# JuliaLinearAlgebra/ArnoldiMethod.jl

Measured on AMD Instinct MI355X. Metric: arnoldi_iters_per_sec, higher is better.
Workload: dtype f64

## Files before the change

arnoldimethod.jl_amd/csrc/ks_csr_layout.hpp:

```cpp
#pragma once

#include <algorithm>
#include <climits>
#include <cmath>
#include <cstring>
#include <unordered_map>
#include <vector>

#include "ks_host_defs.hpp"

namespace {

enum class CbMode {
  None,
  Allowed,
  IsColumnBlock,
  DistributedRowBlock
};

struct FormatRequest {
  bool format_set = false;
  std::string format;
  bool ptr64 = false;
  int sell_sigma = 1;
// ... 35 lines not shown
  bool sell_keeps_dict() const { return format != "sell"; }
};

template <class D> struct CsrHost {
  int64_t nrows, nnz;
  const std::vector<int64_t>& rp;
  const std::vector<int32_t>& ci;
  const std::vector<D>& vv;
};

template <class D> struct CsrPlan {
  int layout = -1;
  bool ptr64 = false;
  double bytes_per_nnz = 0.0, aux_bytes = 0.0;
  int nstencil = 0, nstencil_local = 0, stencil_mask_bytes = 1;
  std::vector<int32_t> sdelta;
  std::vector<D> sval;
  std::vector<uint8_t> mask8;
  std::vector<uint32_t> mask32;
  int ndvi = 0, dvi_unroll = 8, dvi_rpt = 1;
  std::vector<uint8_t> codes;
  std::vector<int32_t> ddelta;
  std::vector<D> dval;
  int ndict = 0;
  std::vector<D> dict;
  std::vector<int32_t> packed;
  int nslices = 0, sell_un = 8;
  int64_t sell_entries = 0;
  std::vector<int64_t> sliceptr;
  std::vector<int32_t> sell_col, sell_perm;
  std::vector<D> sell_val;
  std::vector<CsrPlan<D>> cblocks;
  std::vector<char> cb_from_ghost;
  std::vector<int64_t> cb_bounds;
  int cb_rpt = 0, cb_ni = 0;
  std::vector<int64_t> sub_rp;
  std::vector<int32_t> sub_ci;
  std::vector<D> sub_vv;
  int ni = 7, nblk = 0, nlong = 0;
  bool row_gather = false;
  std::vector<int64_t> blkptr;
  std::vector<int32_t> blkrow, blkpart, lrow, lfirst;
};

template <class D> struct DviDict {
  bool ok = true;
  std::vector<uint8_t> codes;
  std::vector<int32_t> delta;
  std::vector<D> val;
  int64_t max_row = 0;
  std::vector<uint8_t> local_used = std::vector<uint8_t>(256, 0);
};

template <class D> DviDict<D> build_dvi_dict(const CsrHost<D>& A) {
  struct Key {
    uint64_t a, b;
    int64_t d;
    bool operator==(const Key& o) const { return a == o.a && b == o.b && d == o.d; }
  };
  struct KeyHash {
    size_t operator()(const Key& k) const {
      return std::hash<uint64_t>()((k.a * 0x9E3779B97F4A7C15ull ^ k.b) + (uint64_t)k.d * 0xC2B2AE3D27D4EB4Full);
    }
  };
  DviDict<D> t;
  std::unordered_map<Key, int, KeyHash> index;
  t.codes.resize((size_t)A.nnz);
  Key ckey[8];
  int cid[8], ncache = 0, cnext = 0;
  for (int64_t r = 0; r < A.nrows && t.ok; ++r) {
    t.max_row = std::max(t.max_row, A.rp[r + 1] - A.rp[r]);
    for (int64_t p = A.rp[r]; p < A.rp[r + 1]; ++p) {
      Key k{0, 0, (int64_t)A.ci[p] - r};
      std::memcpy(&k, &A.vv[p], sizeof(D));
      bool hit = false;
      for (int q = 0; q < ncache; ++q)
        if (ckey[q] == k) { t.codes[p] = (uint8_t)cid[q]; hit = true; break; }
      if (hit) { if (A.ci[p] < A.nrows) t.local_used[t.codes[p]] = 1; continue; }
      auto it = index.find(k);
      int id;
      if (it == index.end()) {
        if (t.delta.size() == 256) { t.ok = false; break; }
        id = (int)t.delta.size();
        index.emplace(k, id);
        t.delta.push_back((int32_t)k.d);
        t.val.push_back(A.vv[p]);
      } else {
        id = it->second;
      }
      t.codes[p] = (uint8_t)id;
      if (A.ci[p] < A.nrows) t.local_used[id] = 1;
      ckey[cnext] = k;
      cid[cnext] = id;
      cnext = (cnext + 1) & 7;
      if (ncache < 8) ++ncache;
    }
  }
  return t;
}

template <class D> bool plan_stencil(const CsrHost<D>& A, const DviDict<D>& t, CsrPlan<D>& P) {
  const int ns = (int)t.delta.size();
  std::vector<uint32_t> succ((size_t)ns, 0u);
  for (int64_t r = 0; r < A.nrows; ++r)
    for (int64_t p = A.rp[r] + 1; p < A.rp[r + 1]; ++p) succ[t.codes[p - 1]] |= 1u << t.codes[p];
  std::vector<int> indeg((size_t)ns, 0), order;
  for (int a = 0; a < ns; ++a)
    for (int b = 0; b < ns; ++b)
      if (succ[a] >> b & 1u) indeg[b]++;
  std::vector<char> done((size_t)ns, 0);
  for (int it = 0; it < ns; ++it) {
    int pick = -1;
    for (int a = 0; a < ns; ++a)
      if (!done[a] && indeg[a] == 0) { pick = a; break; }
    if (pick < 0) return false;
    done[pick] = 1;
    order.push_back(pick);
    for (int b = 0; b < ns; ++b)
      if (succ[pick] >> b & 1u) indeg[b]--;
  }
  std::vector<int> slot((size_t)ns, 0);
  for (int k = 0; k < ns; ++k) slot[order[k]] = k;
  const int mbytes = ns <= 8 ? 1 : 4;
  std::vector<uint8_t> m8;
  std::vector<uint32_t> m32;
  if (mbytes == 1) m8.assign((size_t)A.nrows, 0); else m32.assign((size_t)A.nrows, 0u);
  for (int64_t r = 0; r < A.nrows; ++r) {
    uint32_t m = 0;
    int last = -1;
    for (int64_t p = A.rp[r]; p < A.rp[r + 1]; ++p) {
      const int k = slot[t.codes[p]];
      if (k <= last) return false;
      last = k;
      m |= 1u << k;
    }
    if (mbytes == 1) m8[r] = (uint8_t)m; else m32[r] = m;
  }
  P.nstencil = ns;
  P.nstencil_local = ns;
  for (int k = ns - 1; k >= 0 && !t.local_used[order[k]]; --k) P.nstencil_local = k;
  P.stencil_mask_bytes = mbytes;
  for (int k = 0; k < ns; ++k) {
    P.sdelta.push_back(t.delta[order[k]]);
    P.sval.push_back(t.val[order[k]]);
  }
  P.mask8 = std::move(m8);
  P.mask32 = std::move(m32);
  P.layout = KS_LAYOUT_STENCIL;
  P.bytes_per_nnz = (double)mbytes * (double)A.nrows / (double)A.nnz;
  P.aux_bytes = 0.0;
  return true;
}

template <class D> void plan_dvi(const CsrHost<D>& A, DviDict<D>&& t, const FormatRequest& req, CsrPlan<D>& P) {
  P.ndvi = (int)t.delta.size();
  P.dvi_unroll = t.max_row <= 4 ? 4 : 8;
  P.dvi_rpt = req.dvi_rpt;
  P.codes = std::move(t.codes);
  P.ddelta = std::move(t.delta);
  P.dval = std::move(t.val);
  P.layout = KS_LAYOUT_DVI;
  P.bytes_per_nnz = 1.0;
  P.aux_bytes = (P.ptr64 ? 8.0 : 4.0) * (double)(A.nrows + 1);
}

template <class D> void build_vi_dict(const CsrHost<D>& A, CsrPlan<D>& P) {
  struct Key {
    uint64_t a, b;
    bool operator==(const Key& o) const { return a == o.a && b == o.b; }
  };
  struct KeyHash {
    size_t operator()(const Key& k) const { return std::hash<uint64_t>()(k.a * 0x9E3779B97F4A7C15ull ^ k.b); }
  };
  std::unordered_map<Key, int, KeyHash> index;
  Key last_key{0, 0};
  int last_id = 0;
  bool ok = true;
  std::vector<D> dict;
  std::vector<int32_t> packed((size_t)A.nnz);
  for (int64_t p = 0; p < A.nnz && ok; ++p) {
    Key k{0, 0};
    std::memcpy(&k, &A.vv[p], sizeof(D));
    int id;
    if (p > 0 && k == last_key) {
      id = last_id;
    } else {
      auto it = index.find(k);
      if (it == index.end()) {
        if (dict.size() == 256) { ok = false; break; }
        id = (int)dict.size();
        index.emplace(k, id);
        dict.push_back(A.vv[p]);
      } else {
        id = it->second;
      }
      last_key = k;
      last_id = id;
    }
    if (A.ci[p] >= (1 << 24)) { ok = false; break; }
    packed[p] = (int32_t)(((uint32_t)id << 24) | (uint32_t)A.ci[p]);
  }
  if (!ok) return;
  P.dict = std::move(dict);
  P.packed = std::move(packed);
  P.ndict = (int)P.dict.size();
}

template <class D> bool plan_sell(const CsrHost<D>& A, const FormatRequest& req, CsrPlan<D>& P) {
  const std::vector<int64_t>& rp = A.rp;
  const int64_t nrows = A.nrows;
  const int sigma = req.sell_sigma;
  std::vector<int32_t> perm;
  if (sigma > 1) {
    perm.resize((size_t)nrows);
    for (int64_t i = 0; i < nrows; ++i) perm[i] = (int32_t)i;
    for (int64_t w0 = 0; w0 < nrows; w0 += sigma) {
      const int64_t w1 = std::min<int64_t>(nrows, w0 + sigma);
      std::stable_sort(perm.begin() + w0, perm.begin() + w1,
                       [&](int32_t x_, int32_t y_) { return rp[x_ + 1] - rp[x_] > rp[y_ + 1] - rp[y_]; });
    }
  }
  auto row_at = [&](int64_t pos) { return sigma > 1 ? (int64_t)perm[pos] : pos; };
  const int64_t nsl = (nrows + 63) / 64;
  std::vector<int64_t> sp((size_t)nsl + 1, 0);
  int64_t wmax = 0;
  for (int64_t sl = 0; sl < nsl; ++sl) {
    int64_t w = 0;
    for (int64_t pos = sl * 64; pos < std::min<int64_t>(nrows, sl * 64 + 64); ++pos) {
      const int64_t r = row_at(pos);
      w = std::max(w, rp[r + 1] - rp[r]);
    }
    wmax = std::max(wmax, w);
    sp[sl + 1] = sp[sl] + 64 * w;
  }
  const int64_t padded = sp[nsl];
  if (!(req.force_sell() || (double)padded <= 1.15 * (double)A.nnz + 64.0)) return false;
  KS_REQUIRE(padded < ((int64_t)1 << 40), KS_ERR_ARGUMENT, "sliced-ELLPACK padding explodes: use KS_SPMV_FORMAT=csr");
  if (padded >= (int64_t)2147483647) P.ptr64 = true;
  const bool vi = P.ndict > 0;
  P.sell_col.assign((size_t)padded, -1);
  P.sell_val.resize(vi ? 0 : (size_t)padded);
  for (int64_t sl = 0; sl < nsl; ++sl)
    for (int64_t pos = sl * 64; pos < std::min<int64_t>(nrows, sl * 64 + 64); ++pos) {
      const int64_t r = row_at(pos);
      const int64_t lane = pos - sl * 64;
      for (int64_t p = rp[r], k = 0; p < rp[r + 1]; ++p, ++k) {
        const int64_t q = sp[sl] + k * 64 + lane;
        P.sell_col[q] = vi ? P.packed[p] : A.ci[p];
        if (!vi) P.sell_val[q] = A.vv[p];
      }
    }
  P.nslices = (int)nsl;
  P.sell_un = wmax <= 4 ? 4 : 8;
  P.sell_entries = padded;
  P.sliceptr = std::move(sp);
  P.sell_perm = std::move(perm);
  P.layout = vi ? KS_LAYOUT_SELL_VI : KS_LAYOUT_SELL;
  P.bytes_per_nnz = (vi ? 4.0 : 4.0 + sizeof(D)) * (double)padded / (double)A.nnz;
  P.aux_bytes = (P.ptr64 ? 8.0 : 4.0) * (double)(nsl + 1) + (sigma > 1 ? 4.0 * (double)nrows : 0.0);
  return true;
}

template <class D> void plan_row_blocks(const CsrHost<D>& A, const FormatRequest& req, CsrPlan<D>& P) {
  const std::vector<int64_t>& rp = A.rp;
  const int64_t nrows = A.nrows;
  constexpr int kBlock = ksd::kBlock;
  const int nimax = (int)(ksd::kSpmvCapBytes / (kBlock * sizeof(D)));
  std::vector<int64_t> tile_nnz;
  for (int64_t r0 = 0; r0 < nrows; r0 += ksd::kSpmvRows) tile_nnz.push_back(rp[std::min<int64_t>(nrows, r0 + ksd::kSpmvRows)] - rp[r0]);
  int64_t t90 = 0;
  if (!tile_nnz.empty()) {
    const size_t k = (tile_nnz.size() - 1) * 9 / 10;
    std::nth_element(tile_nnz.begin(), tile_nnz.begin() + k, tile_nnz.end());
    t90 = tile_nnz[k];
  }
  const int need = (int)((t90 + kBlock - 1) / kBlock);
  int ni = need <= 4 ? 4 : need <= 7 ? 7 : need <= 8 ? 8 : need <= 12 ? 12 : 16;
  if (req.ni != INT_MIN) ni = req.ni;
  if (ni != 4 && ni != 7 && ni != 8 && ni != 12 && ni != 16) ni = 16;
  ni = std::min(ni, nimax);
  P.ni = ni;
  {
    int64_t pairs = 0, close = 0;
    const int64_t stride = std::max<int64_t>(1, nrows / 65536);
    for (int64_t r = 0; r + 1 < nrows; r += stride) {
      if (rp[r + 1] == rp[r] || rp[r + 2] == rp[r + 1]) continue;
      ++pairs;
      const int64_t d = (int64_t)A.ci[rp[r + 1]] - (int64_t)A.ci[rp[r]];
      if (d >= -16 && d <= 16) ++close;
    }
    P.row_gather = req.row_gather >= 0 ? req.row_gather != 0 : (pairs > 0 && 2 * close >= pairs);
  }
  const int64_t cap = (int64_t)ni * kBlock;
  std::vector<int64_t>& bp = P.blkptr;
  std::vector<int32_t>&br = P.blkrow, &part = P.blkpart, &lrow = P.lrow, &lfirst = P.lfirst;
  bp = {0};
  br = {0};
  lfirst = {0};
  int64_t r = 0;
  while (r < nrows) {
    const int64_t first = rp[r + 1] - rp[r];
    if (first > cap) {
      for (int64_t q = rp[r]; q < rp[r + 1]; q += cap) {
        part.push_back((int32_t)lfirst.back() + (int32_t)((q - rp[r]) / cap));
        br.push_back((int32_t)(r + 1));
        bp.push_back(std::min(q + cap, rp[r + 1]));
// ... 172 lines not shown
```

arnoldimethod.jl_amd/csrc/ks_operators.hpp:

```cpp
#pragma once
struct ks_operator {
  ks_ctx* ctx = nullptr;
  int64_t n_local = 0, nnz = 0;
  int dtype = KS_F64;
  bool async_capable = true;
  double bytes_per_nnz = 0.0;
  double aux_bytes = 0.0;
  int layout = -1;
  double in_scale = 1.0;
  bool shift_store_cacheable = false;
  virtual ~ks_operator() = default;
  virtual void apply(const void* x, void* y, const DevState* st) = 0;
  virtual void apply_shifted(const void* x, void* y, double theta_re, double theta_im, double sigma, int64_t ld, const DevState* st);
};

namespace {

template <class D> struct CsrOp : ks_operator {
  void* rowptr = nullptr;
  bool ptr64 = false;
  int32_t* colidx = nullptr;
  D* val = nullptr;
  void* blkptr = nullptr;
  int32_t* blkrow = nullptr;
  int nblk = 0;
  std::vector<std::unique_ptr<CsrOp<D>>> cblocks;
  std::vector<char> cb_from_ghost;
  int cb_rpt = 0, cb_ni = 0;
  int ni = 7;
  bool row_gather = false;
  int nlong = 0;
  int32_t* blkpart = nullptr;
  D* lpart = nullptr;
  int32_t* lrow = nullptr;
  int32_t* lfirst = nullptr;
  int nstencil = 0;
  int stencil_mask_bytes = 1;
  void* smask = nullptr;
  void* smask2 = nullptr;
  ksd::StencilDict<D> sdict{};
  int nstencil_local = 0;
  mutable bool split_said = false;
  void* sliceptr = nullptr;
  int32_t* sperm = nullptr;
  int nslices = 0;
  int sell_un = 8;
  int64_t sell_entries = 0;
  int ndict = 0;
  int ndvi = 0;
  uint8_t* codes = nullptr;
  int32_t* ddelta = nullptr;
  int dvi_unroll = 8;
  int dvi_rpt = 1;
  Halo<D> halo;

  ~CsrOp() override {
    (void)hipFree(rowptr); (void)hipFree(colidx); (void)hipFree(val); (void)hipFree(blkptr); (void)hipFree(blkrow); (void)hipFree(smask); (void)hipFree(sliceptr); (void)hipFree(sperm); (void)hipFree(blkpart); (void)hipFree(lpart); (void)hipFree(lrow); (void)hipFree(lfirst);
    (void)hipFree(codes); (void)hipFree(ddelta);
  }
  void launch_csr_blocks(const D* x, D* y, const DevState* st, const D* yacc, int plain_store, ksd::ShiftArg<D> shift = ksd::ShiftArg<D>{}) {
    hipStream_t s = ctx->stream;
    auto go = [&](auto ip_tag) {
      using IP = decltype(ip_tag);
      auto launch = [&](auto ni_tag) {
        constexpr int NI = decltype(ni_tag)::value;
        if constexpr ((size_t)NI * kBlock * sizeof(D) <= (size_t)ksd::kSpmvCapBytes)
          ksd::k_spmv_csr<D, IP, false, NI><<<nblk, kBlock, 0, s>>>(static_cast<const IP*>(blkptr), blkrow, static_cast<const IP*>(rowptr), colidx, val, x,
                                                                    nullptr, y, n_local, nblk, st, nullptr, 0, 0, nullptr, nullptr, yacc, plain_store,
                                                                    ksd::HaloFused{}, ksd::HaloArgs{}, ksd::P2pDev{}, env_int("KS_SPMV_CSR_NT", 1) != 0, row_gather,
                                                                    plain_store ? ksd::ShiftArg<D>{} : shift);
        else
          throw KsError{KS_ERR_INTERNAL, "CSR row blocks of " + std::to_string(NI) + " x 256 entries exceed the LDS budget of this element type"};
      };
      switch (ni) {
        case 4: launch(std::integral_constant<int, 4>{}); break;
        case 7: launch(std::integral_constant<int, 7>{}); break;
        case 8: launch(std::integral_constant<int, 8>{}); break;
        case 12: launch(std::integral_constant<int, 12>{}); break;
        default: launch(std::integral_constant<int, 16>{}); break;
      }
    };
    if (ptr64) go(int64_t{});
    else go(int32_t{});
  }
  bool shift_on = false;
  D shift_theta{};
  double shift_sigma = 1.0;
  bool shift_plain() const {
    static const int env = env_int("KS_SHIFT_PLAIN", -1);
    return env >= 0 ? env != 0 : shift_store_cacheable;
  }
  static bool march_on() {
    return env_int("KS_STENCIL_MARCH", 1) != 0;
  }
  int march_slots(int ntiles) const {
    const int env = env_int("KS_MARCH_S", 0);
    int S = 192;
    if (env > 0) S = env;
    else {
      int64_t P = 0;
      for (int k = 0; k < nstencil; ++k) P = std::max<int64_t>(P, std::llabs((long long)sdict.delta[k]));
      const int64_t per = P / 512 + 1;
      if (per >= 16 && per <= 224) S = (int)(per * ((160 + per - 1) / per)) <= 224 ? (int)(per * ((160 + per - 1) / per)) : (int)per;
    }
    S = std::min(S, std::max(1, (ntiles + 7) / 8));
    return S;
  }
  void launch_march(const D* x, D* y, int nt, const DevState* st, hipStream_t s) const {
    if constexpr (std::is_same<D, double>::value) {
      const int sh = shift_on ? (1 | (shift_plain() ? 2 : 0)) : 0;
      const uint16_t* m2 = static_cast<const uint16_t*>(smask2);
      const int G = 8 * march_slots(nt);
      int kown = -1;
      for (int k = 0; k < nstencil; ++k)
        if (sdict.delta[k] == 0) kown = k;
      auto go = [&](auto ns_tag, auto ko_tag) {
        ksd::k_spmv_stencil_march<decltype(ns_tag)::value, decltype(ko_tag)::value><<<G, kBlock, 0, s>>>(m2, sdict, x, y, n_local, nt, st, sh, shift_theta, shift_sigma);
      };
      const int window = env_int("KS_MARCH_WINDOW", 1);
      if (window && nstencil == 7 && kown == 3) {
        bool shape = std::llabs((long long)sdict.delta[0]) > 256 && std::llabs((long long)sdict.delta[6]) > 256;
        unsigned odd = 0;
        for (int k = 1; k <= 5; ++k) {
          shape = shape && std::llabs((long long)sdict.delta[k]) <= 256;
          if (sdict.delta[k] & 1) odd |= 1u << k;
        }
        const int zmarch = env_int("KS_MARCH_Z", 1), zr_env = env_int("KS_MARCH_ZR", 0);
        const int64_t Pz = sdict.delta[6];
        if (shape && zmarch && sdict.delta[0] == -Pz && (Pz & 1) == 0 && Pz >= 8 * 8 * 512) {
          const int nzp = (int)((n_local + Pz - 1) / Pz), cmax = (int)(((Pz + 511) / 512 + 7) / 8);
          int nzr = zr_env > 0 ? zr_env : std::max(1, (288 + cmax / 2) / cmax);
          nzr = std::max(1, std::min(nzr, nzp / 4));
          if (nzp >= 8) {
            auto gz = [&](auto odd_tag) {
              ksd::k_spmv_stencil_marchz<7, 0x3eu, decltype(odd_tag)::value, 3, 0, 6><<<8 * cmax * nzr, kBlock, 0, s>>>(m2, sdict, x, y, n_local, nzr, st, sh, shift_theta, shift_sigma);
            };
            if (odd == 0x14u) gz(std::integral_constant<unsigned, 0x14u>{});
            else if (odd == 0x36u) gz(std::integral_constant<unsigned, 0x36u>{});
            else gz(std::integral_constant<unsigned, 0x3eu>{});
            return;
          }
        }
        if (shape) {
          auto gw = [&](auto odd_tag) {
            ksd::k_spmv_stencil_marchw<7, 0x3eu, decltype(odd_tag)::value, 3><<<G, kBlock, 0, s>>>(m2, sdict, x, y, n_local, nt, st, sh, shift_theta, shift_sigma);
          };
          if (odd == 0x14u) gw(std::integral_constant<unsigned, 0x14u>{});
          else if (odd == 0x36u) gw(std::integral_constant<unsigned, 0x36u>{});
          else gw(std::integral_constant<unsigned, 0x3eu>{});
          return;
        }
      }
      using M1 = std::integral_constant<int, -1>;
      if (nstencil == 7 && kown == 3) go(std::integral_constant<int, 7>{}, std::integral_constant<int, 3>{});
      else if (nstencil == 5 && kown == 2) go(std::integral_constant<int, 5>{}, std::integral_constant<int, 2>{});
      else if (nstencil == 3 && kown == 1) go(std::integral_constant<int, 3>{}, std::integral_constant<int, 1>{});
      else switch (nstencil) {
        case 1: go(std::integral_constant<int, 1>{}, M1{}); break;
        case 2: go(std::integral_constant<int, 2>{}, M1{}); break;
        case 3: go(std::integral_constant<int, 3>{}, M1{}); break;
        case 4: go(std::integral_constant<int, 4>{}, M1{}); break;
        case 5: go(std::integral_constant<int, 5>{}, M1{}); break;
        case 6: go(std::integral_constant<int, 6>{}, M1{}); break;
        case 7: go(std::integral_constant<int, 7>{}, M1{}); break;
        default: go(std::integral_constant<int, 8>{}, M1{}); break;
      }
    }
  }
  ksd::ShiftArg<D> shift_arg() const {
    ksd::ShiftArg<D> a;
    a.on = shift_on ? 1 : 0;
    a.theta = shift_theta;
    a.sigma = shift_sigma;
    return a;
  }
  void apply_shifted(const void* xv, void* yv, double tre, double tim, double sigma, int64_t ld, const DevState* st) override {
    const int fuse = env_int("KS_SHIFT_FUSED", 1);
    const bool fused = fuse && n_local > 0 && nlong == 0;
    if (!fused) { ks_operator::apply_shifted(xv, yv, tre, tim, sigma, ld, st); return; }
    shift_on = true;
    if constexpr (sizeof(D) == 8) shift_theta = tre; else shift_theta = D{tre, tim};
    shift_sigma = sigma;
    try { apply(xv, yv, st); } catch (...) { shift_on = false; throw; }
    shift_on = false;
  }
  void apply(const void* xv, void* yv, const DevState* st) override {
    const D* x = static_cast<const D*>(xv);
    D* y = static_cast<D*>(yv);
    hipStream_t s = ctx->stream;
    const typename Halo<D>::Begun begun = halo.begin(x, st, n_local > 0 && cblocks.empty() && ndvi == 0 && nslices == 0);
    const ksd::HaloFused& hf = begun.hf;
    const D* xg = begun.xg;
    if (n_local > 0 && !cblocks.empty()) {
      ProfScope ps(ctx, KSP_SPMV, (double)nnz * bytes_per_nnz + aux_bytes + 2.0 * sizeof(D) * n_local);
      if (cb_rpt) {
        ksd::CbArgs<D> a{};
        a.nb = (int)cblocks.size();
        for (int b = 0; b < a.nb; ++b) {
          a.rowptr[b] = static_cast<const int32_t*>(cblocks[b]->rowptr);
          a.colidx[b] = cblocks[b]->colidx;
          a.val[b] = cblocks[b]->val;
          a.xb[b] = (!cb_from_ghost.empty() && cb_from_ghost[b]) ? xg : nullptr;
        }
        const int nt = (int)((n_local + (int64_t)kBlock * cb_rpt - 1) / ((int64_t)kBlock * cb_rpt));
        auto go = [&](auto ni_tag, auto rpt_tag) {
          constexpr int NI = decltype(ni_tag)::value, RPT = decltype(rpt_tag)::value;
          if constexpr ((size_t)NI * kBlock * sizeof(D) <= (size_t)ksd::kSpmvCapBytes)
            ksd::k_spmv_csr_cb<D, NI, RPT><<<nt, kBlock, 0, s>>>(a, x, y, n_local, nt, st, shift_arg());
          else
            throw KsError{KS_ERR_INTERNAL, "column-blocked CSR: LDS depth exceeds the budget of this element type"};
        };
        auto by_rpt = [&](auto ni_tag) {
          switch (cb_rpt) {
            case 1: go(ni_tag, std::integral_constant<int, 1>{}); break;
            case 2: go(ni_tag, std::integral_constant<int, 2>{}); break;
            case 4: go(ni_tag, std::integral_constant<int, 4>{}); break;
            case 8: go(ni_tag, std::integral_constant<int, 8>{}); break;
            default: go(ni_tag, std::integral_constant<int, 16>{}); break;
          }
        };
        if (cb_ni == 8) by_rpt(std::integral_constant<int, 8>{});
        else by_rpt(std::integral_constant<int, 16>{});
        KS_HIP(hipGetLastError());
        return;
      }
      for (size_t b = 0; b < cblocks.size(); ++b) cblocks[b]->launch_csr_blocks(x, y, st, b > 0 ? y : nullptr, b + 1 < cblocks.size() ? 1 : 0, shift_arg());
      KS_HIP(hipGetLastError());
      return;
    }
    if (n_local > 0) {
      ProfScope ps(ctx, KSP_SPMV, (double)nnz * bytes_per_nnz + aux_bytes + 2.0 * sizeof(D) * n_local);
      const uint32_t* hseq = nullptr;
      auto with_ip = [&](auto f) {
        if (ptr64) f(int64_t{});
        else f(int32_t{});
      };
      if (nstencil > 0 && halo.plan.nghost == 0 && smask2 && n_local >= 2 && env_int("KS_STENCIL_PAIRS", 1)) {
        const int nt = (int)(((n_local + 1) / 2 + kBlock - 1) / kBlock);
        if constexpr (std::is_same<D, double>::value) {
          if (stencil_mask_bytes == 1 && nstencil <= 8 && march_on()) {
            launch_march(x, y, nt, st, s);
            KS_HIP(hipGetLastError());
            return;
          }
        }
        if (stencil_mask_bytes == 1)
          ksd::k_spmv_stencil2<D, uint16_t><<<nt, kBlock, 0, s>>>(static_cast<const uint16_t*>(smask2), sdict, nstencil, x, y, n_local, nt, st, shift_on ? (1 | (shift_plain() ? 2 : 0)) : 0, shift_theta, shift_sigma);
        else
          ksd::k_spmv_stencil2<D, uint64_t><<<nt, kBlock, 0, s>>>(static_cast<const uint64_t*>(smask2), sdict, nstencil, x, y, n_local, nt, st, shift_on ? (1 | (shift_plain() ? 2 : 0)) : 0, shift_theta, shift_sigma);
        KS_HIP(hipGetLastError());
        return;
      }
      if (nstencil > 0 && halo.plan.nghost > 0 && !halo.p2p && smask2 && (stencil_mask_bytes == 1 || stencil_mask_bytes == 4) && n_local >= 2 * kBlock) {
        if constexpr (std::is_same<D, double>::value) {
          static const int split_env = env_int("KS_DIST_SPLIT", 1);
          const int nt1 = (int)((n_local + kBlock - 1) / kBlock);
          const int nlow = (int)((halo.plan.ghost_lo_end + kBlock - 1) / kBlock), first_high = (int)(halo.plan.ghost_hi_begin / kBlock);
          const int nhigh = nt1 - first_high;
          if (split_env && env_int("KS_STENCIL_PAIRS", 1) && nlow <= first_high && 4 * (nlow + nhigh) <= nt1 && nlow + nhigh > 0) {
            const int nt2 = (int)(((n_local + 1) / 2 + kBlock - 1) / kBlock);
            static const int split_dbg = env_int("KS_DIST_SPLIT_DEBUG", 0);
            if (split_dbg && !split_said) {
              split_said = true;
              std::fprintf(stderr, "[split] rows %lld: paired kernel on all of them (%d of %d slots), ghost-aware kernel on %d + %d boundary tiles of %d\n", (long long)n_local, nstencil_local, nstencil, nlow, nhigh, nt1);
            }
            const int shf = shift_on ? (1 | (shift_plain() ? 2 : 0)) : 0;
            ksd::HaloFused h0{};
            const int nsl = nstencil_local >= 1 ? nstencil_local : nstencil;
            if (stencil_mask_bytes == 1) {
              ksd::k_spmv_stencil2<D, uint16_t><<<nt2, kBlock, 0, s>>>(static_cast<const uint16_t*>(smask2), sdict, nsl, x, y, n_local, nt2, st, shf, shift_theta, shift_sigma);
              ksd::k_spmv_stencil<D, uint8_t, 1><<<nlow + nhigh, kBlock, 0, s>>>(static_cast<const uint8_t*>(smask), sdict, nstencil, x, xg, y, n_local,
                                                                                std::max<int64_t>(halo.plan.nghost, 0), nlow + nhigh, st, h0, halo.hargs, ctx->p2p.dev, shift_on ? 1 : 0,
                                                                                shift_theta, shift_sigma, nlow, first_high - nlow);
            } else {
              ksd::k_spmv_stencil2<D, uint64_t><<<nt2, kBlock, 0, s>>>(static_cast<const uint64_t*>(smask2), sdict, nsl, x, y, n_local, nt2, st, shf, shift_theta, shift_sigma);
              ksd::k_spmv_stencil<D, uint32_t, 1><<<nlow + nhigh, kBlock, 0, s>>>(static_cast<const uint32_t*>(smask), sdict, nstencil, x, xg, y, n_local,
                                                                                 std::max<int64_t>(halo.plan.nghost, 0), nlow + nhigh, st, h0, halo.hargs, ctx->p2p.dev, shift_on ? 1 : 0,
                                                                                 shift_theta, shift_sigma, nlow, first_high - nlow);
            }
            KS_HIP(hipGetLastError());
            return;
          }
        }
// ... 117 lines not shown
    KS_HIP(hipGetLastError());
  }
};

struct HostCallbackOp : ks_operator {
  ks_host_apply_fn fn = nullptr;
  void* user = nullptr;
  void* xh = nullptr;
  void* yh = nullptr;
  ~HostCallbackOp() override { (void)hipHostFree(xh); (void)hipHostFree(yh); }
  void apply(const void* x, void* y, const DevState*) override {
    const size_t bytes = (size_t)n_local * (dtype == KS_F64 ? 8 : 16);
    KS_HIP(hipMemcpyAsync(xh, x, bytes, hipMemcpyDeviceToHost, ctx->stream));
    KS_HIP(hipStreamSynchronize(ctx->stream));
    const int64_t nd = n_local * (dtype == KS_F64 ? 1 : 2);
    if (in_scale != 1.0) {
      double* xd = static_cast<double*>(xh);
      for (int64_t i = 0; i < nd; ++i) xd[i] *= in_scale;
    }
    const int rc = fn(user, xh, yh);
    KS_REQUIRE(rc == 0, KS_ERR_OPERATOR, "host operator callback returned " + std::to_string(rc));
    if (in_scale != 1.0) {
      const double back = 1.0 / in_scale;
      double* yd = static_cast<double*>(yh);
      for (int64_t i = 0; i < nd; ++i) yd[i] *= back;
    }
    KS_HIP(hipMemcpyAsync(y, yh, bytes, hipMemcpyHostToDevice, ctx->stream));
  }
};

struct DeviceCallbackOp : ks_operator {
  ks_device_apply_fn fn = nullptr;
  void* user = nullptr;
  void apply(const void* x, void* y, const DevState*) override {
    const int rc = fn(user, x, y, (void*)ctx->stream);
    KS_REQUIRE(rc == 0, KS_ERR_OPERATOR, "device operator callback returned " + std::to_string(rc));
  }
};

template <class I> inline int64_t idx_at(const void* p, int64_t i) { return (int64_t) static_cast<const I*>(p)[i]; }

template <class D>
void build_csr_host(int64_t nrows, int64_t ncols, int64_t nnz, const void* ptr, const void* idx, const void* val,
                    int layout, int base, int itype, std::vector<int64_t>& rp, std::vector<int32_t>& ci,
                    std::vector<D>& vv) {
  auto P = [&](int64_t i) { return (itype == KS_I32 ? idx_at<int32_t>(ptr, i) : idx_at<int64_t>(ptr, i)) - base; };
  auto J = [&](int64_t i) { return (itype == KS_I32 ? idx_at<int32_t>(idx, i) : idx_at<int64_t>(idx, i)) - base; };
  const D* v = static_cast<const D*>(val);
  KS_REQUIRE(nrows < (int64_t)2147483647 && ncols < (int64_t)2147483647, KS_ERR_ARGUMENT, "matrix order must fit int32");
  {
    const int64_t np = (layout == KS_CSR ? nrows : ncols);
    int64_t prev = P(0);
    KS_REQUIRE(prev == 0, KS_ERR_ARGUMENT, layout == KS_CSR ? "row pointer does not match nnz" : "column pointer does not match nnz");
    for (int64_t i = 1; i <= np; ++i) {
      const int64_t cur = P(i);
      KS_REQUIRE(cur >= prev && cur <= nnz, KS_ERR_ARGUMENT, "pointer array is not monotone within [0, nnz]");
      prev = cur;
    }
    KS_REQUIRE(prev == nnz, KS_ERR_ARGUMENT, layout == KS_CSR ? "row pointer does not match nnz" : "column pointer does not match nnz");
  }
  rp.assign(nrows + 1, 0);
  ci.resize(nnz);
  vv.resize(nnz);
  if (layout == KS_CSR) {
    for (int64_t i = 0; i <= nrows; ++i) rp[i] = P(i);
    for (int64_t p = 0; p < nnz; ++p) {
      const int64_t c = J(p);
      KS_REQUIRE(c >= 0 && c < ncols, KS_ERR_ARGUMENT, "column index out of range");
      ci[p] = (int32_t)c;
      vv[p] = v[p];
    }
  } else {
    for (int64_t p = 0; p < nnz; ++p) {
      const int64_t r = J(p);
      KS_REQUIRE(r >= 0 && r < nrows, KS_ERR_ARGUMENT, "row index out of range");
      rp[r + 1]++;
    }
    for (int64_t i = 0; i < nrows; ++i) rp[i + 1] += rp[i];
    std::vector<int64_t> fill(rp.begin(), rp.end() - 1);
    for (int64_t c = 0; c < ncols; ++c)
      for (int64_t p = P(c); p < P(c + 1); ++p) {
        const int64_t r = J(p);
        const int64_t q = fill[r]++;
        ci[q] = (int32_t)c;
        vv[q] = v[p];
      }
  }
}

inline void build_csr_dist_host(int64_t nrows, int64_t nghost, int64_t nnz, const int64_t* rowptr, const int32_t* colidx,
                                std::vector<int64_t>& rp, std::vector<int32_t>& ci) {
  KS_REQUIRE(nrows < (int64_t)2147483647 && nghost < (int64_t)2147483647 - nrows, KS_ERR_ARGUMENT, "local-extended column range must fit int32");
  rp.resize(nrows + 1);
  KS_REQUIRE(rowptr[0] == 0 && rowptr[nrows] == nnz, KS_ERR_ARGUMENT, "row pointer does not match nnz");
  for (int64_t i = 0; i <= nrows; ++i) {
    KS_REQUIRE(i == 0 || (rowptr[i] >= rowptr[i - 1] && rowptr[i] <= nnz), KS_ERR_ARGUMENT, "pointer array is not monotone within [0, nnz]");
    rp[i] = rowptr[i];
  }
  ci.assign(colidx, colidx + nnz);
  for (int64_t p = 0; p < nnz; ++p)
    KS_REQUIRE(ci[p] >= 0 && ci[p] < nrows + nghost, KS_ERR_ARGUMENT, "local-extended column index out of range");
}

inline void* upload_ptr(const std::vector<int64_t>& v, bool ptr64) {
  void* d = nullptr;
  const size_t cnt = v.size();
  if (ptr64) {
    KS_HIP(hipMalloc(&d, std::max<size_t>(cnt * 8, 16)));
    KS_HIP(hipMemcpy(d, v.data(), cnt * 8, hipMemcpyHostToDevice));
  } else {
    std::vector<int32_t> t(v.begin(), v.end());
    KS_HIP(hipMalloc(&d, std::max<size_t>(cnt * 4, 16)));
    KS_HIP(hipMemcpy(d, t.data(), cnt * 4, hipMemcpyHostToDevice));
  }
  return d;
}

template <class T> T* upload_vec(const T* v, size_t cnt, size_t pad, bool zero = false) {
  void* d = nullptr;
  KS_HIP(hipMalloc(&d, (cnt + pad) * sizeof(T)));
  if (zero) KS_HIP(hipMemset(d, 0, (cnt + pad) * sizeof(T)));
  if (cnt) KS_HIP(hipMemcpy(d, v, cnt * sizeof(T), hipMemcpyHostToDevice));
  return static_cast<T*>(d);
}
template <class T> T* upload_vec(const std::vector<T>& v, size_t pad, bool zero = false) { return upload_vec(v.data(), v.size(), pad, zero); }

template <class D>
CsrOp<D>* upload(ks_ctx* ctx, const CsrPlan<D>& P, int64_t nrows, int64_t nnz, const std::vector<int64_t>& rp, const std::vector<int32_t>& ci,
                 const std::vector<D>& vv) {
  auto op = std::make_unique<CsrOp<D>>();
  op->ctx = ctx;
  op->n_local = nrows;
  op->nnz = nnz;
  op->dtype = sizeof(D) == 8 ? KS_F64 : KS_C64;
  op->layout = P.layout;
  op->ptr64 = P.ptr64;
  op->bytes_per_nnz = P.bytes_per_nnz;
  op->aux_bytes = P.aux_bytes;
  op->ndict = P.ndict;
  constexpr size_t kPad16 = 16 / sizeof(D);
  switch (P.layout) {
    case KS_LAYOUT_STENCIL: {
      op->nstencil = P.nstencil;
      op->nstencil_local = P.nstencil_local;
      op->stencil_mask_bytes = P.stencil_mask_bytes;
      for (int k = 0; k < ksd::kStencilSlots; ++k) {
        op->sdict.delta[k] = k < P.nstencil ? P.sdelta[k] : 0;
        op->sdict.val[k] = k < P.nstencil ? P.sval[k] : D{};
      }
      const size_t pad = (size_t)(round_up(nrows + 2, 8) - nrows);
      if (P.stencil_mask_bytes == 1) op->smask = upload_vec(P.mask8, pad, true);
      else op->smask = upload_vec(P.mask32, pad, true);
      op->smask2 = op->smask;
      break;
    }
    case KS_LAYOUT_DVI:
      op->ndvi = P.ndvi;
      op->dvi_unroll = P.dvi_unroll;
      op->dvi_rpt = P.dvi_rpt;
      op->rowptr = upload_ptr(rp, P.ptr64);
      op->codes = upload_vec(P.codes, 64, true);
      op->ddelta = upload_vec(P.ddelta, 256 - P.ddelta.size());
      op->val = upload_vec(P.dval, 256 - P.dval.size());
      break;
    case KS_LAYOUT_SELL:
    case KS_LAYOUT_SELL_VI:
      op->nslices = P.nslices;
      op->sell_un = P.sell_un;
      op->sell_entries = P.sell_entries;
      op->sliceptr = upload_ptr(P.sliceptr, P.ptr64);
      op->colidx = upload_vec(P.sell_col, 4);
      if (P.ndict > 0) op->val = upload_vec(P.dict, 256 - P.dict.size());
      else op->val = upload_vec(P.sell_val, kPad16);
      if (!P.sell_perm.empty()) op->sperm = upload_vec(P.sell_perm, 0);
      break;
    case KS_LAYOUT_CSR_CB:
      for (const CsrPlan<D>& cb : P.cblocks)
        op->cblocks.emplace_back(upload<D>(ctx, cb, nrows, (int64_t)cb.sub_ci.size(), cb.sub_rp, cb.sub_ci, cb.sub_vv));
      op->cb_from_ghost = P.cb_from_ghost;
      op->cb_rpt = P.cb_rpt;
      op->cb_ni = P.cb_ni;
      break;
    default: {
      op->ni = P.ni;
      op->row_gather = P.row_gather;
      op->nlong = P.nlong;
      op->nblk = P.nblk;
      op->blkptr = upload_ptr(P.blkptr, P.ptr64);
      op->blkrow = upload_vec(P.blkrow, P.blkrow.size() < 4 ? 4 - P.blkrow.size() : 0);
      if (P.nlong > 0) {
        op->blkpart = upload_vec(P.blkpart, 0);
        KS_HIP(hipMalloc(&op->lpart, (size_t)P.lfirst.back() * sizeof(D)));
        op->lrow = upload_vec(P.lrow, 0);
        op->lfirst = upload_vec(P.lfirst, 0);
      }
      op->rowptr = upload_ptr(rp, P.ptr64);
      if (P.ndict > 0) {
        op->colidx = upload_vec(P.packed, 2 + 4);
        op->val = upload_vec(P.dict, 256 - P.dict.size());
      } else {
        op->colidx = upload_vec(ci.data(), (size_t)nnz, 2 + 4);
        op->val = upload_vec(vv.data(), (size_t)nnz, 2 + kPad16);
      }
    }
  }
  return op.release();
}

template <class D>
CsrOp<D>* make_csr(ks_ctx* ctx, int64_t nrows, int64_t nnz, const std::vector<int64_t>& rp, const std::vector<int32_t>& ci,
                   const std::vector<D>& vv, CbMode cb_mode = CbMode::None, int64_t nghost = 0, int64_t nlow = 0) {
  const CsrPlan<D> plan = plan_csr<D>(CsrHost<D>{nrows, nnz, rp, ci, vv}, FormatRequest::from_env(), cb_mode, nghost, nlow, ctx->num_cu);
  return upload<D>(ctx, plan, nrows, nnz, rp, ci, vv);
}

}

inline void ks_operator::apply_shifted(const void* x, void* y, double theta_re, double theta_im, double sigma, int64_t ld, const DevState* st) {
  apply(x, y, st);
  ProfScope ps(ctx, KSP_SCALE, 3.0 * (double)n_local * (dtype == KS_F64 ? 8.0 : 16.0));
  const int nbk = (int)std::max<int64_t>(1, std::min<int64_t>((int64_t)ctx->num_cu * 8, ld / (2 * kBlock) + 1));
  if (dtype == KS_F64) {
    ksd::k_shift_scale<double><<<nbk, kBlock, 0, ctx->stream>>>(static_cast<double*>(y), static_cast<const double*>(x), theta_re, sigma, ld, st);
  } else {
    ksd::k_shift_scale<cd><<<nbk, kBlock, 0, ctx->stream>>>(static_cast<cd*>(y), static_cast<const cd*>(x), cd{theta_re, theta_im}, sigma, ld, st);
  }
  KS_HIP(hipGetLastError());
}
```

arnoldimethod.jl_amd/csrc/ks_spmv_march.hpp:

```cpp
#pragma once

#include <algorithm>
#include <type_traits>

#include "ks_kernels.hpp"

namespace ksd {

typedef double f64x2m __attribute__((ext_vector_type(2)));

__device__ __forceinline__ double and_mask(double p, int bm) {
  const uint64_t u = __builtin_bit_cast(uint64_t, p);
  const uint32_t lo = (uint32_t)u & (uint32_t)bm, hi = (uint32_t)(u >> 32) & (uint32_t)bm;
  return __builtin_bit_cast(double, ((uint64_t)hi << 32) | lo);
}

__device__ __forceinline__ int march_tile(int xcd, int slot, int it, int S, int ntiles, int& tend) {
  const int q = ntiles >> 3, r = ntiles & 7;
  const int t0 = xcd < r ? xcd * (q + 1) : r * (q + 1) + (xcd - r) * q;
  tend = t0 + (xcd < r ? q + 1 : q);
  return t0 + slot + it * S;
}

__device__ __forceinline__ void march_ld16(f64x2m& dst, uint32_t voff, const void* sbase) {
// ... 385 lines not shown
  const bool plain_st = (shifted & 2) != 0;
  const bool lane_in = off0 + 2 * (int64_t)threadIdx.x + 1 < P;
  const int nst = (off0 + 128 * (int64_t)wave + 1 < P) ? 1 : 0;
  auto r0_of = [&](int z) { return (int64_t)z * P + off0; };
  auto win_ok = [&](int z) { const int64_t r0 = r0_of(z); return z >= 0 && r0 - 256 >= 0 && r0 + kTile + 256 <= n; };
  auto interior = [&](int z) { return win_ok(z) && r0_of(z) + kTile <= n && (win_ok(z + 1) || r0_of(z + 1) >= n); };

  auto edge = [&](int z) {
    const int64_t r = r0_of(z) + 2 * (int64_t)threadIdx.x;
    if (!lane_in || r >= n) return;
    const bool two = r + 1 < n;
    const uint32_t m = mask2[r >> 1];
    const uint32_t m0 = m & 0xffu, m1 = m >> 8;
    const int64_t cmax = n - 2;
    double s0 = 0.0, s1 = 0.0;
#pragma unroll
    for (int k = 0; k < NSLOT; ++k) {
      const int64_t c = r + d.delta[k];
      int64_t lo = c < 0 ? 0 : (c > cmax ? cmax : c);
      if (cmax < 0) lo = 0;
      const int sh = (int)(c - lo);
      double xa, xb;
      if (n >= 2) ld_pair_u(x + lo, xa, xb);
      else { xa = x[0]; xb = x[0]; }
      const double v0 = sh == 1 ? xb : xa, v1 = sh == -1 ? xa : xb;
      const double p0 = mul_nc(d.val[k], v0), p1 = mul_nc(d.val[k], v1);
      s0 = ((m0 >> k) & 1u) ? add_(s0, p0) : s0;
      s1 = ((m1 >> k) & 1u) ? add_(s1, p1) : s1;
    }
    if (shifted) {
      double x0, x1;
      if (two) ld_pair_u(x + r, x0, x1);
      else { x0 = x[r]; x1 = x0; }
      s0 = scl(sub_s(s0, mul_(theta, x0)), sigma);
      s1 = scl(sub_s(s1, mul_(theta, x1)), sigma);
    }
    if (two) {
      if (plain_st) st_pack(y + r, make_double2(s0, s1));
      else st_pack_nt(y + r, make_double2(s0, s1));
    } else {
      if (plain_st) y[r] = s0;
      else st_elem_nt(y + r, s0);
    }
  };
  int zi0 = za, zi1 = zb;
  while (zi0 < zi1 && !interior(zi0)) ++zi0;
  while (zi1 > zi0 && !interior(zi1 - 1)) --zi1;
  if (zi0 > za || zi1 < zb) {
    for (int z = za; z < zb; ++z)
      if (z < zi0 || z >= zi1) edge(z);
    asm volatile("s_waitcnt vmcnt(0)" ::: "memory");
  }
  if (zi0 >= zi1) return;

  auto issue_w = [&](int zz, int zsafe, int buf) {
    const int zu = win_ok(zz) ? zz : zsafe;
    const double* bw = x + (r0_of(zu) - 256 + (int64_t)wave * 128);
    uint32_t ldst = win0 + (uint32_t)buf * (uint32_t)kWinB + (uint32_t)wave * 1024u;
    asm volatile("" : "+s"(bw));
    asm volatile("" : "+s"(ldst));
    asm volatile("s_nop 4" ::: "memory");
    march_glds16(lane_w, bw, ldst);
    if (wave + kWaves < kPieces) march_glds16(lane_w + (uint32_t)kWaves * 1024u, bw, ldst + (uint32_t)kWaves * 1024u);
  };
  auto issue_m = [&](int zz, uint32_t& m) {
    const uint16_t* bm = mask2 + (r0_of(zz) >> 1);
    asm volatile("" : "+s"(bm));
    asm volatile("s_nop 4" ::: "memory");
    march_ld_u16(m, lane_m, bm);
  };
  f64x2m prev;
  {
    const double* bp = x + (zi0 >= 1 ? r0_of(zi0 - 1) : r0_of(zi0));
    asm volatile("" : "+s"(bp));
    asm volatile("s_nop 4" ::: "memory");
    march_ld16(prev, lane_b, bp);
  }
  uint32_t mA, mB;
  issue_w(zi0, zi0, 0);
  issue_w(zi0 + 1, zi0, 1);
  if constexpr (NB == 4) issue_w(zi0 + 2, zi0, 2);
  issue_m(zi0, mA);
  int bc = 0;
  auto step = [&](int z, uint32_t& m, uint32_t& mnext, bool first, bool has_next) {
    constexpr int NW_LATE = NB == 4 ? 2 : 0;
    if (first) asm volatile("s_waitcnt vmcnt(0)\n\ts_barrier" ::: "memory");
    else if (nst == 0) asm volatile("s_waitcnt vmcnt(%0)\n\ts_barrier" :: "n"(NW_LATE) : "memory");
    else asm volatile("s_waitcnt vmcnt(%0)\n\ts_barrier" :: "n"(NW_LATE + 1) : "memory");
    asm volatile("" : "+v"(m));
    if (first) asm volatile("" : "+v"(prev));
    const int bn = bc + 1 == NB ? 0 : bc + 1, b2 = bc == 0 ? NB - 1 : bc - 1;
    if constexpr (NB == 3) {
      issue_w(z + 2, z, b2);
      if (has_next) issue_m(z + 1, mnext);
    } else {
      if (has_next) issue_m(z + 1, mnext);
      issue_w(z + 3, z, b2);
    }
    const unsigned char* w = &win[0][0] + bc * kWinB + (256 * 8) + threadIdx.x * 16;
    f64x2m v[NSLOT];
#pragma unroll
    for (int k = 0; k < NSLOT; ++k) {
      if ((NEARM >> k) & 1u) {
        const int off = (int)d.delta[k] * 8;
        if (((ODDM >> k) & 1u) == 0) {
          v[k] = *reinterpret_cast<const f64x2m*>(w + off);
        } else {
          typedef double f64x2u8 __attribute__((ext_vector_type(2), aligned(8)));
          const f64x2u8 p = *reinterpret_cast<const f64x2u8*>(w + off);
          v[k].x = p.x;
          v[k].y = p.y;
        }
      }
    }
    v[KFM] = prev;
    v[KFP] = *reinterpret_cast<const f64x2m*>(&win[0][0] + bn * kWinB + (256 * 8) + threadIdx.x * 16);
    const int m0 = (int)(m & 0xffu), m1 = (int)(m >> 8);
    double s0 = 0.0, s1 = 0.0;
#pragma unroll
    for (int k = 0; k < NSLOT; ++k) {
      const double p0 = mul_nc(d.val[k], v[k].x), p1 = mul_nc(d.val[k], v[k].y);
      s0 = add_(s0, and_mask(p0, __builtin_amdgcn_sbfe(m0, k, 1)));
      s1 = add_(s1, and_mask(p1, __builtin_amdgcn_sbfe(m1, k, 1)));
    }
    if (shifted) {
      s0 = scl(sub_s(s0, mul_(theta, v[KOWN].x)), sigma);
      s1 = scl(sub_s(s1, mul_(theta, v[KOWN].y)), sigma);
    }
    prev = v[KOWN];
    f64x2m o2;
    o2.x = s0;
    o2.y = s1;
    double* by = y + r0_of(z);
    asm volatile("" : "+s"(by));
    if (lane_in) march_st16(lane_b, o2, by, plain_st);
    bc = bn;
  };
  int z = zi0;
  bool first = true;
  for (;;) {
    const bool h1 = z + 1 < zi1;
    step(z, mA, mB, first, h1);
    first = false;
    if (!h1) break;
    ++z;
    const bool h2 = z + 1 < zi1;
    step(z, mB, mA, false, h2);
    if (!h2) break;
    ++z;
  }
  asm volatile("s_waitcnt vmcnt(0)" ::: "memory");
}

}
```

Baseline: 4840.

## Skip reloading z-march stencil masks that repeat across planes

At setup, the host compares each 512-row mask tile with the same tile one z-plane earlier and uploads a per-tile repeat bitmap. A new z-marching stencil kernel consults this bitmap and keeps the previous plane's mask registers instead of issuing a new mask load when the masks are identical. It also stops issuing the window prefetch past the last plane, and can optionally process several tiles per block. This removes some mask traffic and loads per plane, at the cost of extra host preprocessing, a small bitmap read, and more complex wait-count and control logic in the kernel.

```diff
diff --git a/arnoldimethod.jl_amd/csrc/ks_csr_layout.hpp b/arnoldimethod.jl_amd/csrc/ks_csr_layout.hpp
--- a/arnoldimethod.jl_amd/csrc/ks_csr_layout.hpp
+++ b/arnoldimethod.jl_amd/csrc/ks_csr_layout.hpp
@@ -211,6 +211,29 @@
   return true;
 }
 
+struct MarchRepeat {
+  int ntiles = 0, nzw = 0;
+  std::vector<uint32_t> bits;
+  bool bit(int t, int z) const { return (bits[(size_t)t * nzw + (z >> 5)] >> (z & 31)) & 1u; }
+};
+inline MarchRepeat plan_march_repeat(const uint16_t* mask2, int64_t n, int64_t P, int nz) {
+  MarchRepeat R;
+  if (P < 2 || (P & 1) || nz < 1) return R;
+  R.ntiles = (int)((P + 511) / 512);
+  R.nzw = (nz + 31) / 32;
+  R.bits.assign((size_t)R.ntiles * R.nzw, 0u);
+  const int64_t half = P / 2;
+  for (int t = 0; t < R.ntiles; ++t) {
+    const int64_t o0 = 512 * (int64_t)t, o1 = std::min<int64_t>(o0 + 512, P);
+    for (int z = 1; z < nz; ++z) {
+      if ((int64_t)z * P + o1 > n) break;
+      const uint16_t* a = mask2 + ((int64_t)z * half + o0 / 2);
+      if (std::memcmp(a, a - half, (size_t)(o1 - o0) / 2 * sizeof(uint16_t)) == 0) R.bits[(size_t)t * R.nzw + (z >> 5)] |= 1u << (z & 31);
+    }
+  }
+  return R;
+}
+
 template <class D> void plan_dvi(const CsrHost<D>& A, DviDict<D>&& t, const FormatRequest& req, CsrPlan<D>& P) {
   P.ndvi = (int)t.delta.size();
   P.dvi_unroll = t.max_row <= 4 ? 4 : 8;
diff --git a/arnoldimethod.jl_amd/csrc/ks_operators.hpp b/arnoldimethod.jl_amd/csrc/ks_operators.hpp
--- a/arnoldimethod.jl_amd/csrc/ks_operators.hpp
+++ b/arnoldimethod.jl_amd/csrc/ks_operators.hpp
@@ -38,6 +38,8 @@
   int stencil_mask_bytes = 1;
   void* smask = nullptr;
   void* smask2 = nullptr;
+  uint32_t* march_rep = nullptr;
+  int march_rep_nzw = 0;
   ksd::StencilDict<D> sdict{};
   int nstencil_local = 0;
   mutable bool split_said = false;
@@ -56,7 +58,7 @@
 
   ~CsrOp() override {
     (void)hipFree(rowptr); (void)hipFree(colidx); (void)hipFree(val); (void)hipFree(blkptr); (void)hipFree(blkrow); (void)hipFree(smask); (void)hipFree(sliceptr); (void)hipFree(sperm); (void)hipFree(blkpart); (void)hipFree(lpart); (void)hipFree(lrow); (void)hipFree(lfirst);
-    (void)hipFree(codes); (void)hipFree(ddelta);
+    (void)hipFree(codes); (void)hipFree(ddelta); (void)hipFree(march_rep);
   }
   void launch_csr_blocks(const D* x, D* y, const DevState* st, const D* yacc, int plain_store, ksd::ShiftArg<D> shift = ksd::ShiftArg<D>{}) {
     hipStream_t s = ctx->stream;
@@ -106,6 +108,11 @@
     S = std::min(S, std::max(1, (ntiles + 7) / 8));
     return S;
   }
+  static constexpr int kMarchMaskReuse = 1, kMarchPpt = 1;
+  bool zmarch_stride(int64_t& Pz) const {
+    Pz = sdict.delta[6];
+    return std::is_same<D, double>::value && nstencil == 7 && stencil_mask_bytes == 1 && sdict.delta[0] == -Pz && (Pz & 1) == 0 && Pz >= 8 * 8 * 512;
+  }
   void launch_march(const D* x, D* y, int nt, const DevState* st, hipStream_t s) const {
     if constexpr (std::is_same<D, double>::value) {
       const int sh = shift_on ? (1 | (shift_plain() ? 2 : 0)) : 0;
@@ -126,9 +133,36 @@
           if (sdict.delta[k] & 1) odd |= 1u << k;
         }
         const int zmarch = env_int("KS_MARCH_Z", 1), zr_env = env_int("KS_MARCH_ZR", 0);
-        const int64_t Pz = sdict.delta[6];
-        if (shape && zmarch && sdict.delta[0] == -Pz && (Pz & 1) == 0 && Pz >= 8 * 8 * 512) {
-          const int nzp = (int)((n_local + Pz - 1) / Pz), cmax = (int)(((Pz + 511) / 512 + 7) / 8);
+        int64_t Pz = 0;
+        if (shape && zmarch && zmarch_stride(Pz)) {
+          const int nzp = (int)((n_local + Pz - 1) / Pz);
+          const int reuse = env_int("KS_MARCH_MASK_REUSE", kMarchMaskReuse) != 0 ? 1 : 0;
+          if (reuse && nzp >= 8 && !march_rep) throw KsError{KS_ERR_INTERNAL, "the z-marching stencil product has no mask-repeat plan"};
+          const int ppt = std::max(1, std::min(3, env_int("KS_MARCH_PPT", kMarchPpt)));
+          const int trim = env_int("KS_MARCH_TRIM", 1) != 0 ? 1 : 0;
+          if (nzp >= 8 && (reuse || ppt > 1)) {
+            const int cmax = (int)(((Pz + 512 * ppt - 1) / (512 * ppt) + 7) / 8);
+            const int per_xcd = ppt == 1 ? 288 : std::max(1, ctx->num_cu / 8) * (ppt == 2 ? 4 : 3);
+            const int nzr = zr_env > 0 ? std::min(zr_env, nzp / 3) : std::max(1, std::min((per_xcd + cmax / 2) / cmax, nzp / 4));
+            auto gp = [&](auto odd_tag, auto ppt_tag, auto reuse_tag) {
+              ksd::k_spmv_stencil_marchzp<7, 0x3eu, decltype(odd_tag)::value, 3, 0, 6, decltype(ppt_tag)::value, decltype(reuse_tag)::value>
+                  <<<8 * cmax * nzr, kBlock, 0, s>>>(m2, sdict, x, y, n_local, nzr, st, sh, shift_theta, shift_sigma, march_rep, march_rep_nzw, trim);
+            };
+            auto gr = [&](auto odd_tag, auto ppt_tag) {
+              if (reuse) gp(odd_tag, ppt_tag, std::true_type{});
+              else gp(odd_tag, ppt_tag, std::false_type{});
+            };
+            auto go_ppt = [&](auto odd_tag) {
+              if (ppt == 1) gr(odd_tag, std::integral_constant<int, 1>{});
+              else if (ppt == 2) gr(odd_tag, std::integral_constant<int, 2>{});
+              else gr(odd_tag, std::integral_constant<int, 3>{});
+            };
+            if (odd == 0x14u) go_ppt(std::integral_constant<unsigned, 0x14u>{});
+            else if (odd == 0x36u) go_ppt(std::integral_constant<unsigned, 0x36u>{});
+            else go_ppt(std::integral_constant<unsigned, 0x3eu>{});
+            return;
+          }
+          const int cmax = (int)(((Pz + 511) / 512 + 7) / 8);
           int nzr = zr_env > 0 ? zr_env : std::max(1, (288 + cmax / 2) / cmax);
           nzr = std::max(1, std::min(nzr, nzp / 4));
           if (nzp >= 8) {
@@ -552,6 +586,14 @@
       if (P.stencil_mask_bytes == 1) op->smask = upload_vec(P.mask8, pad, true);
       else op->smask = upload_vec(P.mask32, pad, true);
       op->smask2 = op->smask;
+      int64_t Pz = 0;
+      if (op->zmarch_stride(Pz) && nrows > 7 * Pz) {
+        std::vector<uint16_t> m2((size_t)(nrows + 1) / 2, 0);
+        std::memcpy(m2.data(), P.mask8.data(), (size_t)nrows);
+        const MarchRepeat R = plan_march_repeat(m2.data(), nrows, Pz, (int)((nrows + Pz - 1) / Pz));
+        op->march_rep = upload_vec(R.bits, 4);
+        op->march_rep_nzw = R.nzw;
+      }
       break;
     }
     case KS_LAYOUT_DVI:
diff --git a/arnoldimethod.jl_amd/csrc/ks_spmv_march.hpp b/arnoldimethod.jl_amd/csrc/ks_spmv_march.hpp
--- a/arnoldimethod.jl_amd/csrc/ks_spmv_march.hpp
+++ b/arnoldimethod.jl_amd/csrc/ks_spmv_march.hpp
@@ -561,4 +561,219 @@
   asm volatile("s_waitcnt vmcnt(0)" ::: "memory");
 }
 
-}
+template <int NSLOT, unsigned NEARM, unsigned ODDM, int KOWN, int KFM, int KFP, int PPT, bool REUSE>
+__global__ void __launch_bounds__(256)
+    k_spmv_stencil_marchzp(const uint16_t* __restrict__ mask2, const StencilDict<double> d, const double* __restrict__ x,
+                           double* __restrict__ y, int64_t n, int nzr, const DevState* __restrict__ st, int shifted, double theta,
+                           double sigma, const uint32_t* __restrict__ rep, int nzw, int trim) {
+  static_assert(KOWN >= 0 && ((NEARM >> KOWN) & 1u) && !((NEARM >> KFM) & 1u) && !((NEARM >> KFP) & 1u), "own pair near, -P / +P far");
+  static_assert(PPT >= 1 && PPT <= 3, "24 / 36 / 48 KiB of windows");
+  if (st && st->breakdown >= 0) return;
+  constexpr int NB = 3, kTile = 512 * PPT, kWinB = (kTile + 512) * 8;
+  __shared__ __attribute__((aligned(16))) unsigned char win[NB][kWinB];
+  const int64_t P = d.delta[KFP];
+  const int nz = (int)((n + P - 1) / P), ntp = (int)((P + kTile - 1) / kTile), ntp512 = (int)((P + 511) / 512);
+  const int xcd = blockIdx.x & 7, slot = blockIdx.x >> 3;
+  int cnt;
+  const int tj0 = march_tile(xcd, 0, 0, 0, ntp, cnt);
+  cnt -= tj0;
+  if (cnt <= 0) return;
+  const int zr = slot / cnt, tile = tj0 + slot % cnt;
+  if (zr >= nzr) return;
+  const int za = (int)((int64_t)zr * nz / nzr), zb = (int)((int64_t)(zr + 1) * nz / nzr);
+  const int64_t off0 = (int64_t)tile * kTile;
+  const uint32_t lane_b = threadIdx.x * 16u, lane_m = threadIdx.x * 2u;
+  const int wave = __builtin_amdgcn_readfirstlane(threadIdx.x >> 6);
+  const uint32_t lane_w = (threadIdx.x & 63u) * 16u;
+  const uint32_t win0 = (uint32_t)(uintptr_t)&win[0][0];
+  const bool plain_st = (shifted & 2) != 0;
+  bool lane_in[PPT];
+  int nst = 0;
+#pragma unroll
+  for (int j = 0; j < PPT; ++j) {
+    lane_in[j] = off0 + 512 * j + 2 * (int64_t)threadIdx.x + 1 < P;
+    nst += (off0 + 512 * j + 128 * (int64_t)wave + 1 < P) ? 1 : 0;
+  }
+  auto r0_of = [&](int z) { return (int64_t)z * P + off0; };
+  auto win_ok = [&](int z) { const int64_t r0 = r0_of(z); return z >= 0 && r0 - 256 >= 0 && r0 + kTile + 256 <= n; };
+  auto interior = [&](int z) { return win_ok(z) && r0_of(z) + kTile <= n && (win_ok(z + 1) || r0_of(z + 1) >= n); };
+
+  auto edge = [&](int z) {
+#pragma unroll
+    for (int j = 0; j < PPT; ++j) {
+      const int64_t r = r0_of(z) + 512 * j + 2 * (int64_t)threadIdx.x;
+      if (!lane_in[j] || r >= n) continue;
+      const bool two = r + 1 < n;
+      const uint32_t m = mask2[r >> 1];
+      const uint32_t m0 = m & 0xffu, m1 = m >> 8;
+      const int64_t cmax = n - 2;
+      double s0 = 0.0, s1 = 0.0;
+#pragma unroll
+      for (int k = 0; k < NSLOT; ++k) {
+        const int64_t c = r + d.delta[k];
+        int64_t lo = c < 0 ? 0 : (c > cmax ? cmax : c);
+        if (cmax < 0) lo = 0;
+        const int sh = (int)(c - lo);
+        double xa, xb;
+        if (n >= 2) ld_pair_u(x + lo, xa, xb);
+        else { xa = x[0]; xb = x[0]; }
+        const double v0 = sh == 1 ? xb : xa, v1 = sh == -1 ? xa : xb;
+        const double p0 = mul_nc(d.val[k], v0), p1 = mul_nc(d.val[k], v1);
+        s0 = ((m0 >> k) & 1u) ? add_(s0, p0) : s0;
+        s1 = ((m1 >> k) & 1u) ? add_(s1, p1) : s1;
+      }
+      if (shifted) {
+        double x0, x1;
+        if (two) ld_pair_u(x + r, x0, x1);
+        else { x0 = x[r]; x1 = x0; }
+        s0 = scl(sub_s(s0, mul_(theta, x0)), sigma);
+        s1 = scl(sub_s(s1, mul_(theta, x1)), sigma);
+      }
+      if (two) {
+        if (plain_st) st_pack(y + r, make_double2(s0, s1));
+        else st_pack_nt(y + r, make_double2(s0, s1));
+      } else {
+        if (plain_st) y[r] = s0;
+        else st_elem_nt(y + r, s0);
+      }
+    }
+  };
+  int zi0 = za, zi1 = zb;
+  while (zi0 < zi1 && !interior(zi0)) ++zi0;
+  while (zi1 > zi0 && !interior(zi1 - 1)) --zi1;
+  if (zi0 > za || zi1 < zb) {
+    for (int z = za; z < zb; ++z)
+      if (z < zi0 || z >= zi1) edge(z);
+    asm volatile("s_waitcnt vmcnt(0)" ::: "memory");
+  }
+  if (zi0 >= zi1) return;
+
+  auto issue_w = [&](int zz, int zsafe, int buf) {
+    const int zu = win_ok(zz) ? zz : zsafe;
+    const double* bw = x + (r0_of(zu) - 256 + (int64_t)wave * 128);
+    uint32_t ldst = win0 + (uint32_t)buf * (uint32_t)kWinB + (uint32_t)wave * 1024u;
+    asm volatile("" : "+s"(bw));
+    asm volatile("" : "+s"(ldst));
+    asm volatile("s_nop 4" ::: "memory");
+#pragma unroll
+    for (int i = 0; i <= PPT; ++i) march_glds16(lane_w + (uint32_t)i * 4096u, bw, ldst + (uint32_t)i * 4096u);
+  };
+  auto issue_m = [&](int zz, uint32_t (&m)[PPT]) {
+    const uint16_t* bm = mask2 + (r0_of(zz) >> 1);
+    asm volatile("" : "+s"(bm));
+    asm volatile("s_nop 4" ::: "memory");
+#pragma unroll
+    for (int j = 0; j < PPT; ++j) march_ld_u16(m[j], lane_m + (uint32_t)j * 512u, bm);
+  };
+  uint32_t rw = 0;
+  int rwi = -1;
+  auto repeats = [&](int zn) -> bool {
+    if constexpr (!REUSE) return false;
+    const int wi = zn >> 5;
+    if (wi != rwi) {
+      rw = ~0u;
+#pragma unroll
+      for (int j = 0; j < PPT; ++j) {
+        const int t5 = tile * PPT + j;
+        if (t5 < ntp512) rw &= rep[(int64_t)t5 * nzw + wi];
+      }
+      rwi = wi;
+    }
+    return ((rw >> (zn & 31)) & 1u) != 0;
+  };
+  f64x2m prev[PPT];
+  {
+    const double* bp = x + (zi0 >= 1 ? r0_of(zi0 - 1) : r0_of(zi0));
+    asm volatile("" : "+s"(bp));
+    asm volatile("s_nop 4" ::: "memory");
+#pragma unroll
+    for (int j = 0; j < PPT; ++j) march_ld16(prev[j], lane_b + (uint32_t)j * 4096u, bp);
+  }
+  uint32_t mA[PPT], mB[PPT];
+  issue_w(zi0, zi0, 0);
+  issue_w(zi0 + 1, zi0, 1);
+  issue_m(zi0, mA);
+  int bc = 0;
+  auto step = [&](int z, uint32_t (&m)[PPT], uint32_t (&mnext)[PPT], bool first, bool has_next, bool load_next) {
+    if (first) asm volatile("s_waitcnt vmcnt(0)\n\ts_barrier" ::: "memory");
+    else if (nst == 0) asm volatile("s_waitcnt vmcnt(0)\n\ts_barrier" ::: "memory");
+    else if (nst == 1) asm volatile("s_waitcnt vmcnt(1)\n\ts_barrier" ::: "memory");
+    else if (nst == 2) asm volatile("s_waitcnt vmcnt(2)\n\ts_barrier" ::: "memory");
+    else asm volatile("s_waitcnt vmcnt(3)\n\ts_barrier" ::: "memory");
+#pragma unroll
+    for (int j = 0; j < PPT; ++j) asm volatile("" : "+v"(m[j]));
+    if (first) {
+#pragma unroll
+      for (int j = 0; j < PPT; ++j) asm volatile("" : "+v"(prev[j]));
+    }
+    const int bn = bc + 1 == NB ? 0 : bc + 1, b2 = bc == 0 ? NB - 1 : bc - 1;
+    if (has_next || !trim) issue_w(z + 2, z, b2);
+    if (load_next) issue_m(z + 1, mnext);
+    double* by = y + r0_of(z);
+    asm volatile("" : "+s"(by));
+#pragma unroll
+    for (int j = 0; j < PPT; ++j) {
+      const unsigned char* w = &win[0][0] + bc * kWinB + (256 * 8) + j * 4096 + threadIdx.x * 16;
+      f64x2m v[NSLOT];
+#pragma unroll
+      for (int k = 0; k < NSLOT; ++k) {
+        if ((NEARM >> k) & 1u) {
+          const int off = (int)d.delta[k] * 8;
+          if (((ODDM >> k) & 1u) == 0) {
+            v[k] = *reinterpret_cast<const f64x2m*>(w + off);
+          } else {
+            typedef double f64x2u8 __attribute__((ext_vector_type(2), aligned(8)));
+            const f64x2u8 p = *reinterpret_cast<const f64x2u8*>(w + off);
+            v[k].x = p.x;
+            v[k].y = p.y;
+          }
+        }
+      }
+      v[KFM] = prev[j];
+      v[KFP] = *reinterpret_cast<const f64x2m*>(&win[0][0] + bn * kWinB + (256 * 8) + j * 4096 + threadIdx.x * 16);
+      const int m0 = (int)(m[j] & 0xffu), m1 = (int)(m[j] >> 8);
+      double s0 = 0.0, s1 = 0.0;
+#pragma unroll
+      for (int k = 0; k < NSLOT; ++k) {
+        const double p0 = mul_nc(d.val[k], v[k].x), p1 = mul_nc(d.val[k], v[k].y);
+        s0 = add_(s0, and_mask(p0, __builtin_amdgcn_sbfe(m0, k, 1)));
+        s1 = add_(s1, and_mask(p1, __builtin_amdgcn_sbfe(m1, k, 1)));
+      }
+      if (shifted) {
+        s0 = scl(sub_s(s0, mul_(theta, v[KOWN].x)), sigma);
+        s1 = scl(sub_s(s1, mul_(theta, v[KOWN].y)), sigma);
+      }
+      prev[j] = v[KOWN];
+      f64x2m o2;
+      o2.x = s0;
+      o2.y = s1;
+      if (lane_in[j]) march_st16(lane_b + (uint32_t)j * 4096u, o2, by, plain_st);
+    }
+    bc = bn;
+  };
+  int z = zi0;
+  bool first = true, more = true;
+  while (more) {
+    for (;;) {
+      const bool h = z + 1 < zi1;
+      const bool ld = h && !repeats(z + 1);
+      step(z, mA, mB, first, h, ld);
+      first = false;
+      ++z;
+      if (!h) more = false;
+      if (!h || ld) break;
+    }
+    if (!more) break;
+    for (;;) {
+      const bool h = z + 1 < zi1;
+      const bool ld = h && !repeats(z + 1);
+      step(z, mB, mA, false, h, ld);
+      ++z;
+      if (!h) more = false;
+      if (!h || ld) break;
+    }
+  }
+  asm volatile("s_waitcnt vmcnt(0)" ::: "memory");
+}
+
+}
```

Result: no change. 4882 (median of 6 runs) (+0.9%).
